# y00njaekim/CMU-11785-IDL-1.58bit-ASR

Hardware: AMD Instinct MI355X
Metric: mel-frames/sec (Conformer-S 1.58-bit train step) (higher is better)
Workload: dtype fp32; 1 GPU; conformer-s-1.58bit-train-step; global_batch=32, execution=hip-graph, per_gpu_batch=32, frames=1000, d_model=144, blocks=16, d_ff=576, heads=4, vocab=5004, parallelism=dp1, passes=teacher 2-bit + student 1-bit + SP, conv_pointwise=fp32 (reference)

## Files before the change

cmu-11785-idl-1.58bit-asr_amd/csrc/capi.hip:

```cpp
#include <algorithm>
#include <vector>

#include "../../include/onebit_hip.h"
#include "ob_launch.h"
#include <stdint.h>

using namespace ob;

namespace {

constexpr int kAbiVersion = 4;

inline hipStream_t as_stream(void* s) { return reinterpret_cast<hipStream_t>(s); }

inline bool aligned4(const void* p) { return (reinterpret_cast<uintptr_t>(p) & 3) == 0; }
inline bool misaligned8(const void* p) { return (reinterpret_cast<uintptr_t>(p) & 7) != 0; }

inline int check_bits(int bits) { return (bits == 1 || bits == 2) ? OB_OK : OB_ERR_BITWIDTH; }

inline int launched() {
  const hipError_t e = hipGetLastError();
  return e == hipSuccess ? OB_OK : OB_ERR_HIP;
}

// ... 970 lines not shown
}

size_t ob_dw_finish_entry_bytes(void) { return sizeof(DwFinishEntry); }

int ob_dw_finish_table(const void* table, int64_t n, int64_t total_blocks, void* stream) {
  if (n < 0 || total_blocks < 0 || total_blocks > 0x7fffffff) return OB_ERR_SHAPE;
  if (n > 0 && !table) return OB_ERR_NULL;
  launch_dw_finish_table(static_cast<const DwFinishEntry*>(table), (int)n, total_blocks,
                         as_stream(stream));
  return launched();
}

int ob_dw_grouped_supported(int64_t N, int64_t K) {
  return N > 0 && K > 0 && N % kDwgTile == 0 && K % kDwgTile == 0 && N <= (1 << 20) &&
         K <= (1 << 20);
}

namespace {
struct DwgPlan {
  std::vector<DwgDesc> d;
  int64_t steps = 0;
  int tiles = 0, blocks = 0;
  size_t table = 0, slots = 0, talpha = 0, total = 0;
};

int dwg_plan(const ob_dwg_gemm* g, int64_t G, DwgPlan& pl) {
  if (G < 1 || G > (1 << 16)) return OB_ERR_SHAPE;
  if (!g) return OB_ERR_NULL;
  pl.d.resize((size_t)G);
  int64_t tiles = 0;
  for (int64_t i = 0; i < G; ++i) {
    const ob_dwg_gemm& e = g[i];
    if (!ob_dw_grouped_supported(e.N, e.K) || e.M < 1 || e.P < 1 || e.P > kMaxPasses ||
        e.M * e.P >= ((int64_t)1 << 30) || e.M * std::max(e.N, e.K) * 4 >= ((int64_t)1 << 31) ||
        e.N * e.K * 4 >= ((int64_t)1 << 31))
      return OB_ERR_SHAPE;
    if (!e.dY || !e.X || !e.dW) return OB_ERR_NULL;
    if (e.W && (!e.alpha || !e.dalpha)) return OB_ERR_NULL;
    if (e.W && !e.pass_bits && check_bits(e.bits) != OB_OK) return OB_ERR_BITWIDTH;
    if (!aligned4(e.dY) || !aligned4(e.X) || ((reinterpret_cast<uintptr_t>(e.dY) |
                                               reinterpret_cast<uintptr_t>(e.X)) & 15))
      return OB_ERR_ALIGN;
    DwgDesc& d = pl.d[(size_t)i];
    d.dY = e.dY;
    d.X = e.X;
    d.W = e.W;
    d.alpha = e.alpha;
    d.pass_bits = e.pass_bits;
    d.dW = e.dW;
    d.db = e.db;
    d.dalpha = e.dalpha;
    d.N = (int)e.N;
    d.K = (int)e.K;
    d.Mp = (int)e.M;
    d.P = (int)e.P;
    d.alpha_raw = e.alpha_raw;
    d.bits = e.bits;
    d.spp = (int)ceil_div(e.M, 32);
    d.tiles_k = (int)(e.K / kDwgTile);
    d.tiles = (int)((e.N / kDwgTile) * d.tiles_k);
    d.tile0 = (int)tiles;
    d.work0 = pl.steps;
    tiles += d.tiles;
    pl.steps += (int64_t)d.tiles * d.P * d.spp;
  }
  if (tiles > (1 << 24) || pl.steps >= ((int64_t)1 << 31)) return OB_ERR_SHAPE;
  pl.tiles = (int)tiles;
  pl.blocks = dwg_blocks(pl.steps);
  pl.table = align_up(sizeof(DwgDesc) * (size_t)G);
  pl.slots = align_up(dwg_slot_bytes() * 2 * (size_t)pl.blocks);
  pl.talpha = align_up(sizeof(float) * (size_t)tiles);
  pl.total = pl.table + pl.slots + pl.talpha;
  return OB_OK;
}
}

size_t ob_dw_grouped_workspace(const ob_dwg_gemm* gemms, int64_t G) {
  DwgPlan pl;
  return dwg_plan(gemms, G, pl) == OB_OK ? pl.total : 0;
}

size_t ob_dw_grouped_tickets(const ob_dwg_gemm* gemms, int64_t G) {
  DwgPlan pl;
  return dwg_plan(gemms, G, pl) == OB_OK ? (size_t)pl.tiles + (size_t)G : 0;
}

int ob_dw_grouped(const ob_dwg_gemm* gemms, int64_t G, void* ws, size_t ws_bytes, void* tickets,
                  size_t ticket_words, void* stream) {
  DwgPlan pl;
  const int st = dwg_plan(gemms, G, pl);
  if (st != OB_OK) return st;
  if (!ws || !tickets) return OB_ERR_NULL;
  if (ws_bytes < pl.total || ticket_words < (size_t)pl.tiles + (size_t)G) return OB_ERR_WORKSPACE;
  unsigned char* base = static_cast<unsigned char*>(ws);
  launch_dw_grouped(pl.d.data(), (int)G, pl.steps, pl.blocks, reinterpret_cast<DwgDesc*>(base),
                    reinterpret_cast<float*>(base + pl.table),
                    reinterpret_cast<float*>(base + pl.table + pl.slots),
                    static_cast<uint32_t*>(tickets), pl.tiles, as_stream(stream));
  return launched();
}

int ob_dwconv1d_fwd(const float* x, const float* w, const float* bias, int64_t B, int64_t C,
                    int64_t T, int64_t KT, float* y, void* stream) {
  if (B < 0 || C < 0 || T < 0 || KT < 1 || KT % 2 == 0 || !dwconv_supported((int)KT))
    return OB_ERR_SHAPE;
  if (B * C * T > 0 && (!x || !y || !w)) return OB_ERR_NULL;
  if (!aligned4(x) || !aligned4(y) || !aligned4(w) || !aligned4(bias)) return OB_ERR_ALIGN;
// ... 1087 lines not shown
```

cmu-11785-idl-1.58bit-asr_amd/csrc/dw.hip:

```cpp
#include <cstdlib>
#include <type_traits>

#include "ob_launch.h"
#include "ob_mma.h"
#include "ob_quant.h"

namespace ob {

namespace {

constexpr int kThreads = 256;

constexpr int kDwTile = 64;

template <bool VEC, int S>
__global__ __launch_bounds__(kThreads) void dw_partial_kernel(
    const float* __restrict__ dY, const float* __restrict__ X, int64_t M, int64_t N, int64_t K,
    int64_t tiles_k, int64_t rows_per_chunk, int64_t cpp, float* __restrict__ part,
    float* __restrict__ part_db, uint32_t* __restrict__ ticket) {
  __shared__ float red[2][kDwTile * kDwTile];
  __shared__ float dbred[4][kDwTile];

  const int lane = threadIdx.x & 63;
  const int wave = threadIdx.x >> 6;
// ... 654 lines not shown
constexpr int kDwgAl = kDwgDb + kDwgTile;
constexpr unsigned kSc1 = 16;

__device__ __forceinline__ int dwg_start(int b, int nb, int W) {
  return (int)((long long)b * W / nb);
}
__device__ __forceinline__ int dwg_owner(int x, int nb, int W) {
  return (int)(((long long)(x + 1) * nb - 1) / W);
}

__device__ __forceinline__ float ld_f32(__amdgpu_buffer_rsrc_t r, int voff) {
  return __builtin_bit_cast(float, __builtin_amdgcn_raw_buffer_load_b32(r, voff, 0, 0));
}
__device__ __forceinline__ void st_f32(float v, __amdgpu_buffer_rsrc_t r, int voff) {
  __builtin_amdgcn_raw_buffer_store_b32(__builtin_bit_cast(uint32_t, v), r, voff, 0, 0);
}

__device__ __forceinline__ int opaque(int x) {
  asm volatile("" : "+v"(x));
  return x;
}

constexpr int kDwgWaves = 8, kDwgThreads = 64 * kDwgWaves;
constexpr int kDwgBuf = 2 * kDwgTile * kLdsPitch;
constexpr int kDwgLds = 2 * kDwgBuf + 16 * kDwgTile * 4 + 16;

__global__ __launch_bounds__(kDwgThreads) void dw_grouped_kernel(
    const DwgDesc* __restrict__ descs, int G, int Wtot, float* __restrict__ slots,
    float* __restrict__ talpha, uint32_t* __restrict__ tickets, int total_tiles) {
  constexpr int BN = kDwgTile;
  extern __shared__ __attribute__((aligned(16))) unsigned char lds[];
  const int lane = threadIdx.x & 63;
  const int wave = __builtin_amdgcn_readfirstlane(threadIdx.x >> 6);
  const int bn = wave / 3, bk = wave - 3 * bn;
  const int tie = 6 + bn, tue = 6 + bk;
  const bool two = wave == 7;
  const int r = lane & 15, g = lane >> 4;
  const int nb = gridDim.x, blk = blockIdx.x;
  const int beg = dwg_start(blk, nb, Wtot), end = dwg_start(blk + 1, nb, Wtot);
  float* const s_db = reinterpret_cast<float*>(lds + 2 * kDwgBuf);
  int* const s_flag = reinterpret_cast<int*>(lds + 2 * kDwgBuf + 16 * kDwgTile * 4);
  float* const fl = reinterpret_cast<float*>(lds);
  const bool u2 = wave == 0;
  const int rp0 = threadIdx.x & 15, cq0 = 4 * (threadIdx.x >> 4);
  const int cq1 = 128 + cq0;

  int gi = 0;
  {
    int lo = 0, hi = G - 1;
    while (lo < hi) {
      const int mid = (lo + hi + 1) >> 1;
      if (descs[mid].work0 <= beg) lo = mid;
      else hi = mid - 1;
    }
    gi = lo;
  }

  auto put = [&](unsigned char* base, int col, const f32x4& r0, const f32x4& r1) {
#pragma unroll
    for (int e = 0; e < 4; ++e) {
      uint32_t ph, pm, pl;
      split2(r0[e], r1[e], ph, pm, pl);
      unsigned char* cb = base + (col + e) * kLdsPitch + rp0 * 4;
      *reinterpret_cast<uint32_t*>(cb) = ph;
      *reinterpret_cast<uint32_t*>(cb + 64) = pm;
      *reinterpret_cast<uint32_t*>(cb + 128) = pl;
    }
  };
  auto frag = [&](const unsigned char* base, int col, int plane) {
    return *reinterpret_cast<const bf16x8*>(base + col * kLdsPitch + 64 * plane + 16 * g);
  };

  int pos = beg;
  while (pos < end) {
    const DwgDesc& d = descs[gi];
    const int tsteps = d.P * d.spp;
    if (pos >= (int)d.work0 + tsteps * d.tiles) {
      ++gi;
      continue;
    }
    const int t = (pos - (int)d.work0) / tsteps;
    const int T0 = (int)d.work0 + t * tsteps, T1 = T0 + tsteps;
    const int send = end < T1 ? end : T1;
    const int N = d.N, K = d.K, Mp = d.Mp, spp = d.spp;
    const int tn = t / d.tiles_k, tk = t - tn * d.tiles_k;
    const int n0 = tn * kDwgTile, k0 = tk * kDwgTile;
    const bool has_al = d.W != nullptr;
    const bool do_db = d.db != nullptr && tk == 0;
    const float a = has_al ? effective_alpha(d.alpha, d.alpha_raw) : 1.0f;
    const __amdgpu_buffer_rsrc_t rw = make_rsrc(d.W, has_al ? (int64_t)N * K * 4 : 0);
    auto pass_bits = [&](int p) {
      const int b = d.pass_bits ? d.pass_bits[p] : d.bits;
      return b == 1 ? 1 : 2;
    };

    f32x4 acc[3][3], acce[2];
#pragma unroll
    for (int i = 0; i < 3; ++i)
#pragma unroll
      for (int u = 0; u < 3; ++u) acc[i][u] = f32x4{0.f, 0.f, 0.f, 0.f};
    acce[0] = acce[1] = f32x4{0.f, 0.f, 0.f, 0.f};
    auto for_tiles = [&](auto&& fn) {
#pragma unroll
      for (int i = 0; i < 3; ++i)
#pragma unroll
        for (int u = 0; u < 3; ++u) fn(acc[i][u], 3 * bn + i, 3 * bk + u);
      fn(acce[0], tie, tue);
      if (two) fn(acce[1], 8, 8);
    };
    auto elem_base = [&]() {
      const int ln = opaque(lane);
      return ((n0 + 4 * (ln >> 4)) * K + k0 + (ln & 15)) * 4;
    };
    float aprod = 0.0f;
    auto alpha_dot = [&](int b1, int b2) {
      const int eb = elem_base();
      for_tiles([&](f32x4& ac, int ti, int tu) {
        float w[4];
#pragma unroll
        for (int reg = 0; reg < 4; ++reg)
          w[reg] = ld_f32(rw, eb + ((16 * ti + reg) * K + 16 * tu) * 4);
#pragma unroll
        for (int reg = 0; reg < 4; ++reg) {
          const float wa = w[reg] / a;
          aprod += ac[reg] * (alpha_term(wa, b1) - (b2 ? alpha_term(wa, b2) : 0.0f));
        }
      });
    };
    f32x4* const db0 = reinterpret_cast<f32x4*>(s_db + rp0 * kDwgTile + cq0);
    f32x4* const db1 = reinterpret_cast<f32x4*>(s_db + rp0 * kDwgTile + cq1);

    __syncthreads();
    if (do_db) {
      *db0 = f32x4{0.f, 0.f, 0.f, 0.f};
      if (u2) *db1 = f32x4{0.f, 0.f, 0.f, 0.f};
    }
    int j = pos - T0;
    const int j1 = send - T0;
    while (j < j1) {
      const int p = j / spp;
      const int je = j1 < (p + 1) * spp ? j1 : (p + 1) * spp;
      const int r0 = p * Mp + (j - p * spp) * kStepRows;
      const int rl = p * Mp + (je - p * spp) * kStepRows;
      const int r1 = rl < (p + 1) * Mp ? rl : (p + 1) * Mp;
      const int steps = je - j;
      const __amdgpu_buffer_rsrc_t ry =
          make_rsrc(d.dY + (int64_t)r0 * N, (int64_t)(r1 - r0) * N * 4);
      const __amdgpu_buffer_rsrc_t rx =
          make_rsrc(d.X + (int64_t)r0 * K, (int64_t)(r1 - r0) * K * 4);
      const __amdgpu_buffer_rsrc_t ry2 = u2 ? ry : make_rsrc(d.dY, 0);
      const __amdgpu_buffer_rsrc_t rx2 = u2 ? rx : make_rsrc(d.X, 0);
      const int yv0 = (2 * rp0 * N + n0 + cq0) * 4, xv0 = (2 * rp0 * K + k0 + cq0) * 4;
      struct Raw {
        f32x4 y[2][2];
        f32x4 x[2][2];
      };
      auto load = [&](Raw& raw, int step) {
        const int soy = step * kStepRows * N * 4, sox = step * kStepRows * K * 4;
#pragma unroll
        for (int i = 0; i < 2; ++i) {
          raw.y[0][i] = __builtin_amdgcn_raw_buffer_load_b128(ry, yv0, soy + i * N * 4, 0);
          raw.x[0][i] = __builtin_amdgcn_raw_buffer_load_b128(rx, xv0, sox + i * K * 4, 0);
        }
#pragma unroll
        for (int i = 0; i < 2; ++i) {
          raw.y[1][i] = __builtin_amdgcn_raw_buffer_load_b128(ry2, yv0 + 512, soy + i * N * 4, 0);
          raw.x[1][i] = __builtin_amdgcn_raw_buffer_load_b128(rx2, xv0 + 512, sox + i * K * 4, 0);
        }
      };
      auto store = [&](const Raw& raw, int buf) {
        unsigned char* base = lds + buf * kDwgBuf;
        if (do_db) *db0 = *db0 + (raw.y[0][0] + raw.y[0][1]);
        put(base, cq0, raw.y[0][0], raw.y[0][1]);
        put(base, BN + cq0, raw.x[0][0], raw.x[0][1]);
        if (u2) {
          if (do_db) *db1 = *db1 + (raw.y[1][0] + raw.y[1][1]);
          put(base, cq1, raw.y[1][0], raw.y[1][1]);
          put(base, BN + cq1, raw.x[1][0], raw.x[1][1]);
        }
      };
      auto compute = [&](int buf) {
        const unsigned char* base = lds + buf * kDwgBuf;
        bf16x8 bq[3][3];
#pragma unroll
        for (int u = 0; u < 3; ++u)
#pragma unroll
          for (int q = 0; q < 3; ++q) bq[u][q] = frag(base, BN + 48 * bk + 16 * u + r, q);
#pragma unroll
        for (int i = 0; i < 3; ++i) {
          bf16x8 aq[3];
#pragma unroll
          for (int q = 0; q < 3; ++q) aq[q] = frag(base, 48 * bn + 16 * i + r, q);
#pragma unroll
          for (int pr = 0; pr < 6; ++pr)
#pragma unroll
            for (int u = 0; u < 3; ++u)
              acc[i][u] = mfma_bf16(aq[kProdA[pr]], bq[u][kProdB[pr]], acc[i][u]);
        }
        bf16x8 ae[3], be[3];
#pragma unroll
        for (int q = 0; q < 3; ++q) ae[q] = frag(base, 16 * tie + r, q);
#pragma unroll
        for (int q = 0; q < 3; ++q) be[q] = frag(base, BN + 16 * tue + r, q);
#pragma unroll
        for (int pr = 0; pr < 6; ++pr) acce[0] = mfma_bf16(ae[kProdA[pr]], be[kProdB[pr]], acce[0]);
        if (two) {
#pragma unroll
          for (int q = 0; q < 3; ++q) be[q] = frag(base, BN + 16 * 8 + r, q);
#pragma unroll
          for (int pr = 0; pr < 6; ++pr)
            acce[1] = mfma_bf16(ae[kProdA[pr]], be[kProdB[pr]], acce[1]);
        }
      };
      auto phase = [&](int cb, Raw& nxt, int sb, bool do_store, int ld_step) {
        (void)do_store;
        store(nxt, sb);
        compute(cb);
        load(nxt, ld_step);
      };
      Raw ra, rb;
      load(ra, 0);
      load(rb, 1);
      store(ra, 0);
      load(ra, 2);
      __syncthreads();
      for (int s = 0; s < steps; s += 2) {
        phase(0, rb, 1, true, s + 3);
        __syncthreads();
        phase(1, ra, 0, true, s + 4);
        __syncthreads();
      }
      if (has_al) {
        const int bp = pass_bits(p);
        if (je == j1) {
          alpha_dot(bp, 0);
        } else {
          const int bq = pass_bits(p + 1);
          if (bq != bp) alpha_dot(bp, bq);
        }
      }
      j = je;
    }

    const int tid = opaque((int)threadIdx.x);
    const int ln = tid & 63;
    if (has_al) {
#pragma unroll
      for (int off = 32; off >= 1; off >>= 1) aprod += __shfl_xor(aprod, off, 64);
      if (ln == 0) fl[wave] = aprod;
    }
    __syncthreads();
    float dbv = 0.0f, ap = 0.0f;
    if (do_db && tid < kDwgTile) {
#pragma unroll
      for (int q = 0; q < 16; ++q) dbv += s_db[q * kDwgTile + tid];
    }
    if (has_al && tid == 0) {
      for (int w = 0; w < kDwgWaves; ++w) ap += fl[w];
    }
    auto slab_off = [&](int ti, int tu) { return ((ti * 9 + tu) * 64) * 16; };

    bool finish = pos == T0 && send == T1;
    if (!finish) {
      const int nsl = dwg_owner(T1 - 1, nb, Wtot) - dwg_owner(T0, nb, Wtot) + 1;
      float* slab = slots + (int64_t)(2 * blk + (beg >= T0 ? 0 : 1)) * kDwgSlotF;
      const __amdgpu_buffer_rsrc_t rs = make_rsrc(slab, (int64_t)kDwgSlotF * 4);
      for_tiles([&](f32x4& ac, int ti, int tu) {
        __builtin_amdgcn_raw_buffer_store_b128(ac, rs, ln * 16, slab_off(ti, tu), kSc1);
      });
      if (do_db && tid < kDwgTile)
        __hip_atomic_store(slab + kDwgDb + tid, dbv, __ATOMIC_RELAXED, __HIP_MEMORY_SCOPE_AGENT);
      if (has_al && tid == 0)
        __hip_atomic_store(slab + kDwgAl, ap, __ATOMIC_RELAXED, __HIP_MEMORY_SCOPE_AGENT);
      asm volatile("s_waitcnt vmcnt(0)" ::: "memory");
      __syncthreads();
      if (tid == 0) {
        const uint32_t old = __hip_atomic_fetch_add(tickets + d.tile0 + t, 1u, __ATOMIC_RELAXED,
                                                    __HIP_MEMORY_SCOPE_AGENT);
        *s_flag = old == (uint32_t)(nsl - 1);
      }
      __syncthreads();
      finish = *s_flag != 0;
      if (finish) {
        __builtin_amdgcn_fence(__ATOMIC_ACQUIRE, "wavefront");
        const int bf = dwg_owner(T0, nb, Wtot);
        dbv = 0.0f;
        ap = 0.0f;
        for (int q = 0; q < nsl; ++q) {
          const int bb = bf + q;
          const float* sl =
              slots + (int64_t)(2 * bb + (dwg_start(bb, nb, Wtot) >= T0 ? 0 : 1)) * kDwgSlotF;
          const __amdgpu_buffer_rsrc_t rl = make_rsrc(sl, (int64_t)kDwgSlotF * 4);
          for_tiles([&](f32x4& ac, int ti, int tu) {
            const f32x4 v = __builtin_amdgcn_raw_buffer_load_b128(rl, ln * 16, slab_off(ti, tu), kSc1);
            ac = q == 0 ? v : ac + v;
          });
          if (do_db && tid < kDwgTile) {
            const float v =
                __hip_atomic_load(sl + kDwgDb + tid, __ATOMIC_RELAXED, __HIP_MEMORY_SCOPE_AGENT);
            dbv = q == 0 ? v : dbv + v;
          }
          if (has_al && tid == 0) {
            const float v =
                __hip_atomic_load(sl + kDwgAl, __ATOMIC_RELAXED, __HIP_MEMORY_SCOPE_AGENT);
            ap = q == 0 ? v : ap + v;
          }
        }
        if (tid == 0)
          __hip_atomic_store(tickets + d.tile0 + t, 0u, __ATOMIC_RELAXED, __HIP_MEMORY_SCOPE_AGENT);
      }
    }
    if (finish) {
      const __amdgpu_buffer_rsrc_t rd = make_rsrc(d.dW, (int64_t)N * K * 4);
      const int eb = elem_base();
      for_tiles([&](f32x4& ac, int ti, int tu) {
        float w[4];
        if (has_al) {
#pragma unroll
          for (int reg = 0; reg < 4; ++reg)
            w[reg] = ld_f32(rw, eb + ((16 * ti + reg) * K + 16 * tu) * 4);
        }
#pragma unroll
        for (int reg = 0; reg < 4; ++reg) {
          float v = ac[reg];
          if (has_al) v *= ste_indicator(w[reg] / a);
          st_f32(v, rd, eb + ((16 * ti + reg) * K + 16 * tu) * 4);
        }
      });
      if (do_db && tid < kDwgTile) d.db[n0 + tid] = dbv;
      if (has_al && tid == 0) {
        const float chain = alpha_chain(d.alpha, d.alpha_raw);
        if (d.tiles == 1) {
          *d.dalpha = ap * chain;
        } else {
          __hip_atomic_store(talpha + d.tile0 + t, ap, __ATOMIC_RELAXED, __HIP_MEMORY_SCOPE_AGENT);
          asm volatile("s_waitcnt vmcnt(0)" ::: "memory");
          uint32_t* gt = tickets + total_tiles + gi;
          const uint32_t old =
              __hip_atomic_fetch_add(gt, 1u, __ATOMIC_RELAXED, __HIP_MEMORY_SCOPE_AGENT);
          if (old == (uint32_t)(d.tiles - 1)) {
            __builtin_amdgcn_fence(__ATOMIC_ACQUIRE, "wavefront");
            float s2 = 0.0f;
            for (int q = 0; q < d.tiles; ++q)
              s2 += __hip_atomic_load(talpha + d.tile0 + q, __ATOMIC_RELAXED,
                                      __HIP_MEMORY_SCOPE_AGENT);
            *d.dalpha = s2 * chain;
            __hip_atomic_store(gt, 0u, __ATOMIC_RELAXED, __HIP_MEMORY_SCOPE_AGENT);
          }
        }
      }
    }
    pos = send;
  }
}

constexpr int kDwgChunk = 32;
static_assert(sizeof(DwgDesc) * kDwgChunk + 64 <= 4096, "dwg_table_kernel arguments exceed 4 KiB");
struct DwgChunk {
  DwgDesc d[kDwgChunk];
};
__global__ void dwg_table_kernel(DwgDesc* table, int off, int n, DwgChunk c) {
  if ((int)threadIdx.x < n) table[off + threadIdx.x] = c.d[threadIdx.x];
}


}

DwPlan plan_dw(int64_t M, int64_t N, int64_t K) { return plan_dw_passes(1, M, N, K); }

DwPlan plan_dw_passes(int64_t P, int64_t Mp, int64_t N, int64_t K) {
  DwPlan p;
  const int64_t M = P * Mp;
  if (N % 4 != 0 || K % 4 != 0 || N < 4 || K < 4) {
    p.variant = 0;
    p.tiles_n = N > 0 ? ceil_div(N, kDwTile) : 1;
// ... 116 lines not shown
                   dW, db, dalpha};
  const int64_t nb = finish_blocks(a);
  hipLaunchKernelGGL(dw_finish_kernel, dim3((unsigned)nb), dim3(kThreads), 0, s, a);
}

int64_t dw_finish_blocks(const DwFinish& a) { return finish_blocks(a); }

__global__ void dw_table_entry_kernel(DwFinishEntry* table, int slot, DwFinishEntry ent) {
  table[slot] = ent;
}

void launch_dw_table_entry(DwFinishEntry* table, int slot, const DwFinishEntry& ent,
                           hipStream_t s) {
  hipLaunchKernelGGL(dw_table_entry_kernel, dim3(1), dim3(1), 0, s, table, slot, ent);
}

void launch_dw_finish_table(const DwFinishEntry* table, int n, int64_t total_blocks,
                            hipStream_t s) {
  if (n <= 0 || total_blocks <= 0) return;
  hipLaunchKernelGGL(dw_finish_table_kernel, dim3((unsigned)total_blocks), dim3(kThreads), 0, s,
                     table, n, total_blocks);
}

int dwg_blocks(int64_t total_steps) {
  int dev = 0, cus = 0;
  if (hipGetDevice(&dev) != hipSuccess ||
      hipDeviceGetAttribute(&cus, hipDeviceAttributeMultiprocessorCount, dev) != hipSuccess ||
      cus <= 0)
    cus = 256;
  return (int)(total_steps < cus ? total_steps : cus);
}

size_t dwg_slot_bytes() { return sizeof(float) * (size_t)kDwgSlotF; }

void launch_dw_grouped(const DwgDesc* host_descs, int G, int64_t total_steps, int blocks,
                       DwgDesc* table, float* slots, float* talpha, uint32_t* tickets,
                       int total_tiles, hipStream_t s) {
  for (int off = 0; off < G; off += kDwgChunk) {
    DwgChunk c{};
    const int n = G - off < kDwgChunk ? G - off : kDwgChunk;
    for (int i = 0; i < n; ++i) c.d[i] = host_descs[off + i];
    hipLaunchKernelGGL(dwg_table_kernel, dim3(1), dim3(kDwgChunk), 0, s, table, off, n, c);
  }
  hipLaunchKernelGGL(dw_grouped_kernel, dim3((unsigned)blocks), dim3(kDwgThreads),
                     (size_t)kDwgLds, s, table, G, (int)total_steps, slots,
                     talpha, tickets, total_tiles);
}

void launch_dw_finish_group(const DwFinish* a, int n, hipStream_t s) {
  DwFinishGroup G{};
  G.n = n;
  int64_t total = 0;
  for (int i = 0; i < n; ++i) {
    G.g[i] = a[i];
    G.start[i] = (int)total;
    total += finish_blocks(a[i]);
// ... 14 lines not shown
```

cmu-11785-idl-1.58bit-asr_amd/csrc/ob_launch.h:

```cpp
#pragma once

#include <hip/hip_runtime.h>
#include <stddef.h>
#include <stdint.h>

#include "../../include/onebit_hip.h"

namespace ob {

inline int64_t ceil_div(int64_t a, int64_t b) { return (a + b - 1) / b; }

void launch_quant_pack(const float* W, const float* alpha, int alpha_raw, int bits,
                       const int* bits_dev, int64_t N, int64_t K, uint32_t* codes,
                       uint32_t* codes_t, hipStream_t s);
int64_t quant_pack_item_blocks(int64_t N, int64_t K);
int64_t quant_pack_item_blocks16(int64_t N, int64_t K);
void launch_quant_pack_group(const ob_pack_item* items_dev, int n_items, int64_t total_blocks,
                             hipStream_t s);
void launch_quant_dequant(const float* W, const float* alpha, int alpha_raw, int bits, int64_t n,
                          float* W_hat, hipStream_t s);

int64_t ste_reduce_blocks(int64_t total);
void launch_ste_reduce(const float* part, int chunks, int64_t nk, const float* part_db,
                       int64_t n_db, const float* W, const float* alpha, int alpha_raw, int bits,
// ... 157 lines not shown
};
int64_t dw_finish_blocks(const DwFinish& a);
void launch_dw_table_entry(DwFinishEntry* table, int slot, const DwFinishEntry& ent, hipStream_t s);
void launch_dw_finish_table(const DwFinishEntry* table, int n, int64_t total_blocks, hipStream_t s);
void launch_dw_partial_group_defer(const float* const* dY, int G, const float* X, int64_t M,
                                   int64_t N, int64_t K, const DwPlan& p, float* const* part,
                                   float* const* part_db, const DwAlpha* al,
                                   DwFinishEntry* table, int slot, const DwFinishEntry* ent,
                                   hipStream_t s);

struct DwgDesc {
  const float* dY;
  const float* X;
  const float* W;
  const float* alpha;
  const int* pass_bits;
  float* dW;
  float* db;
  float* dalpha;
  int64_t work0;
  int N, K, Mp, P, alpha_raw, bits;
  int spp;
  int tiles_k;
  int tiles;
  int tile0;
};
constexpr int kDwgTile = 144;
int dwg_blocks(int64_t total_steps);
size_t dwg_slot_bytes();
void launch_dw_grouped(const DwgDesc* host_descs, int G, int64_t total_steps, int blocks,
                       DwgDesc* table, float* slots, float* talpha, uint32_t* tickets,
                       int total_tiles, hipStream_t s);

bool dense_gemm_supported(int64_t K, int64_t N);
struct DenseEpi {
  const float* R;
  float p_drop;
  const uint64_t* rng;
  uint64_t rng_off;
};
bool launch_dense_gemm(const float* A, int64_t M, int64_t K, const float* W, int trans,
                       const float* bias, int64_t N, float* C, hipStream_t s,
                       const DenseEpi* epi = nullptr);

bool ternary_gemm_i8_supported(int64_t K, int64_t N);
void launch_silu_monotone_check(uint32_t lo, uint32_t hi, uint32_t* bad, hipStream_t s);
size_t act_absmax_workspace(int P);
void launch_act_absmax(const float* X, int P, int64_t n_per_pass, float* amax, void* ws,
                       hipStream_t s);
void launch_act_dequant(const float* X, int P, int64_t n_per_pass, const float* amax, float* Xd,
                        hipStream_t s);
// ... 261 lines not shown
```

cmu-11785-idl-1.58bit-asr_amd/onebit_asr/_lib.py:

```python
from __future__ import annotations

import ctypes
import os
from pathlib import Path

import torch

LIB_NAME = "libonebit_hip.so"
LIB_PATH = Path(os.environ.get("ONEBIT_HIP_LIB") or Path(__file__).with_name(LIB_NAME))

OB_OK = 0
OB_ERR_SHAPE = -2
OB_ERR_BITWIDTH = -3

_c_f = ctypes.c_void_p
_i64 = ctypes.c_int64
_int = ctypes.c_int
_sz = ctypes.c_size_t
_f32 = ctypes.c_float
_f64 = ctypes.c_double

SIGNATURES = {
    "ob_abi_version": (_int, []),
    "ob_source_digest": (ctypes.c_char_p, []),
# ... 177 lines not shown
    "ob_layernorm_fwd_i8": (_int, [_c_f, _c_f, _c_f, _i64, _i64, _f32, _i64, _c_f, _c_f, _c_f,
                                   _sz, _c_f]),
    "ob_layernorm_bwd_defer": (
        _int, [_c_f, _c_f, _c_f, _c_f, _c_f, _i64, _i64, _c_f, _c_f, _c_f, _c_f, _c_f, _sz, _c_f,
               _f32, _f32, _c_f, _i64, _c_f, _i64, _c_f, _i64, _c_f]),
    "ob_layernorm_bwd_pair_workspace": (_sz, [_i64, _i64]),
    "ob_layernorm_bwd_pair": (
        _int, [_c_f, _c_f, _c_f, _c_f, _c_f, _c_f, _c_f, _c_f, _c_f, _c_f, _i64, _i64, _c_f, _c_f,
               _c_f, _c_f, _c_f, _c_f, _sz, _c_f, _f32, _f32, _c_f, _i64, _c_f, _i64, _c_f, _i64,
               _i64, _c_f]),
    "ob_ln_param_entry_bytes": (_sz, []),
    "ob_ln_param_table": (_int, [_c_f, _i64, _i64, _c_f]),
    "ob_dw_finish_entry_bytes": (_sz, []),
    "ob_bitlinear_bwd_dw_passes_defer": (
        _int, [_c_f, _c_f, _i64, _i64, _i64, _i64, _c_f, _c_f, _int, _c_f, _c_f, _c_f, _c_f, _c_f,
               _sz, _c_f, _i64, _i64, _c_f, _c_f]),
    "ob_bitlinear_bwd_dw_passes_group_defer": (
        _int, [_i64, _c_f, _c_f, _i64, _i64, _i64, _i64, _c_f, _c_f, _int, _c_f, _c_f, _c_f, _c_f,
               _c_f, _sz, _c_f, _i64, _i64, _c_f, _c_f]),
    "ob_dw_finish_table": (_int, [_c_f, _i64, _i64, _c_f]),
    "ob_dw_grouped_supported": (_int, [_i64, _i64]),
    "ob_dw_grouped_workspace": (_sz, [_c_f, _i64]),
    "ob_dw_grouped_tickets": (_sz, [_c_f, _i64]),
    "ob_dw_grouped": (_int, [_c_f, _i64, _c_f, _sz, _c_f, _sz, _c_f]),
    "ob_dense_dw_defer": (_int, [_c_f, _c_f, _i64, _i64, _i64, _c_f, _c_f, _c_f, _sz, _c_f, _i64,
                                 _i64, _c_f, _c_f]),
    "ob_layernorm_bwd_workspace": (_sz, [_i64, _i64]),
    "ob_layernorm_bwd": (
        _int, [_c_f, _c_f, _c_f, _c_f, _c_f, _i64, _i64, _c_f, _c_f, _c_f, _c_f, _sz, _c_f]),
    "ob_layernorm_bwd_res": (
        _int, [_c_f, _c_f, _c_f, _c_f, _c_f, _i64, _i64, _c_f, _c_f, _c_f, _c_f, _c_f, _sz, _c_f]),
    "ob_layernorm_bwd_ex": (
        _int, [_c_f, _c_f, _c_f, _c_f, _c_f, _i64, _i64, _c_f, _c_f, _c_f, _c_f, _c_f, _sz, _c_f,
               _f32, _f32, _c_f, _i64, _c_f, _i64, _c_f]),
    "ob_act_absmax_workspace": (_sz, [_i64]),
    "ob_act_absmax": (_int, [_c_f, _i64, _i64, _c_f, _c_f, _sz, _c_f]),
    "ob_act_dequant_i8": (_int, [_c_f, _i64, _i64, _c_f, _c_f, _c_f]),
    "ob_bitlinear_fwd_i8": (
        _int, [_c_f, _i64, _i64, _i64, _c_f, _c_f, _c_f, _c_f, _int, _c_f, _c_f, _i64, _c_f, _c_f]),
    "ob_bitlinear_fwd_i8_epi": (
        _int, [_c_f, _i64, _i64, _i64, _c_f, _c_f, _c_f, _c_f, _int, _c_f, _c_f, _i64, _int, _c_f,
               _f32, _c_f, _i64, _c_f, _c_f, _c_f]),
    "ob_bitlinear_fwd_passes_group": (
        _int, [_i64, _c_f, _i64, _i64, _i64, _c_f, _c_f, _c_f, _c_f, _int, _c_f, _i64, _c_f, _c_f]),
    "ob_bitlinear_fwd_i8q": (
        _int, [_c_f, _i64, _i64, _i64, _c_f, _c_f, _c_f, _c_f, _int, _c_f, _c_f, _i64, _int, _c_f,
# ... 108 lines not shown
```

include/onebit_hip.h:

```cpp
#ifndef ONEBIT_HIP_H_
#define ONEBIT_HIP_H_

#include <stddef.h>
#include <stdint.h>

#ifdef __cplusplus
extern "C" {
#endif

#define OB_API __attribute__((visibility("default")))

enum {
  OB_OK = 0,
  OB_ERR_NULL = -1,
  OB_ERR_SHAPE = -2,
  OB_ERR_BITWIDTH = -3,
  OB_ERR_WORKSPACE = -4,
  OB_ERR_ALIGN = -5,
  OB_ERR_HIP = -6
};

OB_API int ob_abi_version(void);
OB_API const char* ob_source_digest(void);
OB_API const char* ob_status_string(int status);
// ... 177 lines not shown
OB_API int ob_bitlinear_bwd_dw_passes_group_defer(
    int64_t G, const float* const* dY, const float* X, int64_t P, int64_t M, int64_t N,
    int64_t K, const float* const* W, const float* const* alpha, int alpha_raw,
    const int32_t* pass_bits, float* const* dW, float* const* dalpha, float* const* db,
    void* ws, size_t ws_bytes, void* table, int64_t slot, int64_t start, int64_t* n_blocks,
    void* stream);
OB_API int ob_dw_finish_table(const void* table, int64_t n, int64_t total_blocks, void* stream);

typedef struct ob_dwg_gemm {
  const float* dY;
  const float* X;
  const float* W;
  const float* alpha;
  const int32_t* pass_bits;
  float* dW;
  float* db;
  float* dalpha;
  int64_t N, K, M, P;
  int32_t alpha_raw, bits;
} ob_dwg_gemm;
OB_API int ob_dw_grouped_supported(int64_t N, int64_t K);
OB_API size_t ob_dw_grouped_workspace(const ob_dwg_gemm* gemms, int64_t G);
OB_API size_t ob_dw_grouped_tickets(const ob_dwg_gemm* gemms, int64_t G);
OB_API int ob_dw_grouped(const ob_dwg_gemm* gemms, int64_t G, void* ws, size_t ws_bytes,
                         void* tickets, size_t ticket_words, void* stream);

OB_API int ob_decattn_supported(int64_t Lq, int64_t Lk, int64_t dh);
OB_API int ob_decattn_fwd(const float* q, int64_t sq, const float* k, int64_t sk, const float* v,
                          int64_t sv, const uint8_t* kmask, int64_t causal, int64_t B, int64_t H,
                          int64_t Lq, int64_t Lk, int64_t dh, float p_drop, const int64_t* rng,
                          int64_t rng_offset, float* probs, float* ctx, void* stream);
OB_API int ob_decattn_bwd(const float* dctx, const float* ctx, const float* q, int64_t sq,
                          const float* k, int64_t sk, const float* v, int64_t sv, int64_t B, int64_t H, int64_t Lq,
                          int64_t Lk, int64_t dh, float p_drop, float* probs, float* dq,
                          int64_t gq, float* dk, int64_t gk, float* dv, int64_t gv, void* stream);
OB_API int ob_decattn_fwd_grouped(const float* q, int64_t sq, const float* k, int64_t sk,
                                  const float* v, int64_t sv, const uint8_t* kmask,
                                  int64_t causal, int64_t B, int64_t kv_group, int64_t H,
                                  int64_t Lq, int64_t Lk, int64_t dh, float* ctx, void* stream);

OB_API int ob_relattn_fwd(const float* q, const float* k, const float* v, const float* pos,
                          const float* u, const float* vb, const int32_t* lens, int64_t Bt,
                          int64_t P, int64_t T, int64_t H, int64_t d, float p_drop,
                          const int64_t* rng, int64_t rng_offset, float* saved, float* probs,
                          float* ctx, void* stream);
OB_API int64_t ob_relattn_saved_elems(int64_t Bt, int64_t T, int64_t H, int64_t d);
// ... 322 lines not shown
```

Baseline: 1.408 million mel-frames/s.

## Pair adjacent dW output tiles in grouped kernel to share one operand load

The grouped weight-gradient kernel now processes pairs of adjacent 144x144 output tiles, along N or along K, as one work unit. The shared operand (X or dY) is loaded into LDS once and reused for both tiles, so each pair streams three operand panels instead of four. This costs a second set of accumulators, double-size split-K slots and bias reduction buffers, more syncs per step, and coarser work units for load balancing. A helper reports the operand bytes read.

```diff
diff --git a/cmu-11785-idl-1.58bit-asr_amd/csrc/capi.hip b/cmu-11785-idl-1.58bit-asr_amd/csrc/capi.hip
--- a/cmu-11785-idl-1.58bit-asr_amd/csrc/capi.hip
+++ b/cmu-11785-idl-1.58bit-asr_amd/csrc/capi.hip
@@ -1016,6 +1016,7 @@
   int64_t steps = 0;
   int tiles = 0, blocks = 0;
   size_t table = 0, slots = 0, talpha = 0, total = 0;
+  size_t operand_bytes = 0;
 };
 
 int dwg_plan(const ob_dwg_gemm* g, int64_t G, DwgPlan& pl) {
@@ -1052,15 +1053,22 @@
     d.bits = e.bits;
     d.spp = (int)ceil_div(e.M, 32);
     d.tiles_k = (int)(e.K / kDwgTile);
-    d.tiles = (int)((e.N / kDwgTile) * d.tiles_k);
+    const DwgPairing pr = dwg_pairing(e.N, e.K);
+    d.pairs = pr.pairs;
+    d.singles = pr.singles;
+    d.kdir = pr.kdir;
     d.tile0 = (int)tiles;
     d.work0 = pl.steps;
-    tiles += d.tiles;
-    pl.steps += (int64_t)d.tiles * d.P * d.spp;
+    const int64_t gt = 2 * (int64_t)pr.pairs + pr.singles;
+    tiles += gt;
+    pl.steps += gt * d.P * d.spp;
+    pl.steps += pl.steps & 1;
+    pl.operand_bytes += (size_t)e.M * e.P * 4 *
+                        ((size_t)pr.pairs * 3 * kDwgTile + (size_t)pr.singles * 2 * kDwgTile);
   }
   if (tiles > (1 << 24) || pl.steps >= ((int64_t)1 << 31)) return OB_ERR_SHAPE;
   pl.tiles = (int)tiles;
-  pl.blocks = dwg_blocks(pl.steps);
+  pl.blocks = dwg_blocks(pl.steps / 2);
   pl.table = align_up(sizeof(DwgDesc) * (size_t)G);
   pl.slots = align_up(dwg_slot_bytes() * 2 * (size_t)pl.blocks);
   pl.talpha = align_up(sizeof(float) * (size_t)tiles);
@@ -1077,6 +1085,11 @@
 size_t ob_dw_grouped_tickets(const ob_dwg_gemm* gemms, int64_t G) {
   DwgPlan pl;
   return dwg_plan(gemms, G, pl) == OB_OK ? (size_t)pl.tiles + (size_t)G : 0;
+}
+
+size_t ob_dw_grouped_operand_bytes(const ob_dwg_gemm* gemms, int64_t G) {
+  DwgPlan pl;
+  return dwg_plan(gemms, G, pl) == OB_OK ? pl.operand_bytes : 0;
 }
 
 int ob_dw_grouped(const ob_dwg_gemm* gemms, int64_t G, void* ws, size_t ws_bytes, void* tickets,
diff --git a/cmu-11785-idl-1.58bit-asr_amd/csrc/dw.hip b/cmu-11785-idl-1.58bit-asr_amd/csrc/dw.hip
--- a/cmu-11785-idl-1.58bit-asr_amd/csrc/dw.hip
+++ b/cmu-11785-idl-1.58bit-asr_amd/csrc/dw.hip
@@ -700,13 +700,17 @@
 }
 
 constexpr int kDwgWaves = 8, kDwgThreads = 64 * kDwgWaves;
-constexpr int kDwgBuf = 2 * kDwgTile * kLdsPitch;
-constexpr int kDwgLds = 2 * kDwgBuf + 16 * kDwgTile * 4 + 16;
+constexpr int kDwgReg = kDwgTile * kLdsPitch;
+constexpr int kDwgBuf = 2 * kDwgReg;
+constexpr int kDwgDbF = 16 * kDwgTile;
+constexpr int kDwgLds = 2 * kDwgBuf + 2 * kDwgDbF * 4 + 16;
 
 __global__ __launch_bounds__(kDwgThreads) void dw_grouped_kernel(
     const DwgDesc* __restrict__ descs, int G, int Wtot, float* __restrict__ slots,
     float* __restrict__ talpha, uint32_t* __restrict__ tickets, int total_tiles) {
   constexpr int BN = kDwgTile;
+  using C0 = std::integral_constant<int, 0>;
+  using C1 = std::integral_constant<int, 1>;
   extern __shared__ __attribute__((aligned(16))) unsigned char lds[];
   const int lane = threadIdx.x & 63;
   const int wave = __builtin_amdgcn_readfirstlane(threadIdx.x >> 6);
@@ -715,9 +719,10 @@
   const bool two = wave == 7;
   const int r = lane & 15, g = lane >> 4;
   const int nb = gridDim.x, blk = blockIdx.x;
-  const int beg = dwg_start(blk, nb, Wtot), end = dwg_start(blk + 1, nb, Wtot);
+  const int H = Wtot >> 1;
+  const int beg = 2 * dwg_start(blk, nb, H), end = 2 * dwg_start(blk + 1, nb, H);
   float* const s_db = reinterpret_cast<float*>(lds + 2 * kDwgBuf);
-  int* const s_flag = reinterpret_cast<int*>(lds + 2 * kDwgBuf + 16 * kDwgTile * 4);
+  int* const s_flag = reinterpret_cast<int*>(lds + 2 * kDwgBuf + 2 * kDwgDbF * 4);
   float* const fl = reinterpret_cast<float*>(lds);
   const bool u2 = wave == 0;
   const int rp0 = threadIdx.x & 15, cq0 = 4 * (threadIdx.x >> 4);
@@ -753,18 +758,42 @@
   while (pos < end) {
     const DwgDesc& d = descs[gi];
     const int tsteps = d.P * d.spp;
-    if (pos >= (int)d.work0 + tsteps * d.tiles) {
+    const int work0 = (int)d.work0;
+    const int pw = 2 * d.pairs * tsteps;
+    if (pos >= work0 + pw + d.singles * tsteps) {
+      if (gi + 1 >= G) break;
       ++gi;
       continue;
     }
-    const int t = (pos - (int)d.work0) / tsteps;
-    const int T0 = (int)d.work0 + t * tsteps, T1 = T0 + tsteps;
+    if (pos < work0) {
+      pos = work0;
+      continue;
+    }
+    auto run_unit = [&](auto pair_c) -> int {
+    constexpr bool pair = decltype(pair_c)::value;
+    const int cost = pair ? 2 : 1;
+    const int t = pair ? (pos - work0) / (2 * tsteps) : d.pairs + (pos - work0 - pw) / tsteps;
+    const int T0 = pair ? work0 + t * 2 * tsteps : work0 + pw + (t - d.pairs) * tsteps;
+    const int T1 = T0 + cost * tsteps;
     const int send = end < T1 ? end : T1;
     const int N = d.N, K = d.K, Mp = d.Mp, spp = d.spp;
-    const int tn = t / d.tiles_k, tk = t - tn * d.tiles_k;
+    const bool kdir = d.kdir != 0;
+    const int tiles_n = N / kDwgTile;
+    int tn, tk;
+    if (pair) {
+      const int pn = kdir ? 1 : tiles_n / 2;
+      tk = kdir ? 2 * t : t / pn;
+      tn = kdir ? 0 : 2 * (t - tk * pn);
+    } else {
+      tn = kdir ? 0 : tiles_n - 1;
+      tk = kdir ? d.tiles_k - 1 : t - d.pairs;
+    }
+    const int units = d.pairs + d.singles;
     const int n0 = tn * kDwgTile, k0 = tk * kDwgTile;
+    const int n0b = n0 + (kdir ? 0 : kDwgTile), k0b = k0 + (kdir ? kDwgTile : 0);
     const bool has_al = d.W != nullptr;
     const bool do_db = d.db != nullptr && tk == 0;
+    const bool do_dbb = do_db && pair && !kdir;
     const float a = has_al ? effective_alpha(d.alpha, d.alpha_raw) : 1.0f;
     const __amdgpu_buffer_rsrc_t rw = make_rsrc(d.W, has_al ? (int64_t)N * K * 4 : 0);
     auto pass_bits = [&](int p) {
@@ -772,38 +801,45 @@
       return b == 1 ? 1 : 2;
     };
 
-    f32x4 acc[3][3], acce[2];
-#pragma unroll
-    for (int i = 0; i < 3; ++i)
-#pragma unroll
-      for (int u = 0; u < 3; ++u) acc[i][u] = f32x4{0.f, 0.f, 0.f, 0.f};
-    acce[0] = acce[1] = f32x4{0.f, 0.f, 0.f, 0.f};
-    auto for_tiles = [&](auto&& fn) {
+    f32x4 acc[2][3][3], acce[2][2];
+#pragma unroll
+    for (int w = 0; w < 2; ++w) {
 #pragma unroll
       for (int i = 0; i < 3; ++i)
 #pragma unroll
-        for (int u = 0; u < 3; ++u) fn(acc[i][u], 3 * bn + i, 3 * bk + u);
-      fn(acce[0], tie, tue);
-      if (two) fn(acce[1], 8, 8);
+        for (int u = 0; u < 3; ++u) acc[w][i][u] = f32x4{0.f, 0.f, 0.f, 0.f};
+      acce[w][0] = acce[w][1] = f32x4{0.f, 0.f, 0.f, 0.f};
+    }
+    auto for_tiles = [&](auto wc, auto&& fn) {
+      constexpr int w = decltype(wc)::value;
+#pragma unroll
+      for (int i = 0; i < 3; ++i)
+#pragma unroll
+        for (int u = 0; u < 3; ++u) fn(acc[w][i][u], 3 * bn + i, 3 * bk + u);
+      fn(acce[w][0], tie, tue);
+      if (two) fn(acce[w][1], 8, 8);
     };
-    auto elem_base = [&]() {
+    auto elem_base = [&](int tn0, int tk0) {
       const int ln = opaque(lane);
-      return ((n0 + 4 * (ln >> 4)) * K + k0 + (ln & 15)) * 4;
+      return ((tn0 + 4 * (ln >> 4)) * K + tk0 + (ln & 15)) * 4;
     };
     float aprod = 0.0f;
     auto alpha_dot = [&](int b1, int b2) {
-      const int eb = elem_base();
-      for_tiles([&](f32x4& ac, int ti, int tu) {
-        float w[4];
-#pragma unroll
-        for (int reg = 0; reg < 4; ++reg)
-          w[reg] = ld_f32(rw, eb + ((16 * ti + reg) * K + 16 * tu) * 4);
-#pragma unroll
-        for (int reg = 0; reg < 4; ++reg) {
-          const float wa = w[reg] / a;
-          aprod += ac[reg] * (alpha_term(wa, b1) - (b2 ? alpha_term(wa, b2) : 0.0f));
-        }
-      });
+      auto one = [&](auto wc, int eb) {
+        for_tiles(wc, [&](f32x4& ac, int ti, int tu) {
+          float w[4];
+#pragma unroll
+          for (int reg = 0; reg < 4; ++reg)
+            w[reg] = ld_f32(rw, eb + ((16 * ti + reg) * K + 16 * tu) * 4);
+#pragma unroll
+          for (int reg = 0; reg < 4; ++reg) {
+            const float wa = w[reg] / a;
+            aprod += ac[reg] * (alpha_term(wa, b1) - (b2 ? alpha_term(wa, b2) : 0.0f));
+          }
+        });
+      };
+      one(C0{}, elem_base(n0, k0));
+      if (pair) one(C1{}, elem_base(n0b, k0b));
     };
     f32x4* const db0 = reinterpret_cast<f32x4*>(s_db + rp0 * kDwgTile + cq0);
     f32x4* const db1 = reinterpret_cast<f32x4*>(s_db + rp0 * kDwgTile + cq1);
@@ -813,8 +849,12 @@
       *db0 = f32x4{0.f, 0.f, 0.f, 0.f};
       if (u2) *db1 = f32x4{0.f, 0.f, 0.f, 0.f};
     }
-    int j = pos - T0;
-    const int j1 = send - T0;
+    if (do_dbb) {
+      db0[kDwgDbF / 4] = f32x4{0.f, 0.f, 0.f, 0.f};
+      if (u2) db1[kDwgDbF / 4] = f32x4{0.f, 0.f, 0.f, 0.f};
+    }
+    int j = (pos - T0) / cost;
+    const int j1 = (send - T0) / cost;
     while (j < j1) {
       const int p = j / spp;
       const int je = j1 < (p + 1) * spp ? j1 : (p + 1) * spp;
@@ -857,56 +897,131 @@
           put(base, BN + cq1, raw.x[1][0], raw.x[1][1]);
         }
       };
-      auto compute = [&](int buf) {
-        const unsigned char* base = lds + buf * kDwgBuf;
+      auto compute = [&](auto wc, const unsigned char* ya, const unsigned char* xa) {
+        constexpr int w = decltype(wc)::value;
         bf16x8 bq[3][3];
 #pragma unroll
         for (int u = 0; u < 3; ++u)
 #pragma unroll
-          for (int q = 0; q < 3; ++q) bq[u][q] = frag(base, BN + 48 * bk + 16 * u + r, q);
+          for (int q = 0; q < 3; ++q) bq[u][q] = frag(xa, 48 * bk + 16 * u + r, q);
 #pragma unroll
         for (int i = 0; i < 3; ++i) {
           bf16x8 aq[3];
 #pragma unroll
-          for (int q = 0; q < 3; ++q) aq[q] = frag(base, 48 * bn + 16 * i + r, q);
+          for (int q = 0; q < 3; ++q) aq[q] = frag(ya, 48 * bn + 16 * i + r, q);
 #pragma unroll
           for (int pr = 0; pr < 6; ++pr)
 #pragma unroll
             for (int u = 0; u < 3; ++u)
-              acc[i][u] = mfma_bf16(aq[kProdA[pr]], bq[u][kProdB[pr]], acc[i][u]);
+              acc[w][i][u] = mfma_bf16(aq[kProdA[pr]], bq[u][kProdB[pr]], acc[w][i][u]);
         }
         bf16x8 ae[3], be[3];
 #pragma unroll
-        for (int q = 0; q < 3; ++q) ae[q] = frag(base, 16 * tie + r, q);
-#pragma unroll
-        for (int q = 0; q < 3; ++q) be[q] = frag(base, BN + 16 * tue + r, q);
-#pragma unroll
-        for (int pr = 0; pr < 6; ++pr) acce[0] = mfma_bf16(ae[kProdA[pr]], be[kProdB[pr]], acce[0]);
+        for (int q = 0; q < 3; ++q) ae[q] = frag(ya, 16 * tie + r, q);
+#pragma unroll
+        for (int q = 0; q < 3; ++q) be[q] = frag(xa, 16 * tue + r, q);
+#pragma unroll
+        for (int pr = 0; pr < 6; ++pr)
+          acce[w][0] = mfma_bf16(ae[kProdA[pr]], be[kProdB[pr]], acce[w][0]);
         if (two) {
 #pragma unroll
-          for (int q = 0; q < 3; ++q) be[q] = frag(base, BN + 16 * 8 + r, q);
+          for (int q = 0; q < 3; ++q) be[q] = frag(xa, 16 * 8 + r, q);
 #pragma unroll
           for (int pr = 0; pr < 6; ++pr)
-            acce[1] = mfma_bf16(ae[kProdA[pr]], be[kProdB[pr]], acce[1]);
+            acce[w][1] = mfma_bf16(ae[kProdA[pr]], be[kProdB[pr]], acce[w][1]);
         }
       };
       auto phase = [&](int cb, Raw& nxt, int sb, bool do_store, int ld_step) {
         (void)do_store;
         store(nxt, sb);
-        compute(cb);
+        compute(C0{}, lds + cb * kDwgBuf, lds + cb * kDwgBuf + kDwgReg);
         load(nxt, ld_step);
       };
-      Raw ra, rb;
-      load(ra, 0);
-      load(rb, 1);
-      store(ra, 0);
-      load(ra, 2);
-      __syncthreads();
-      for (int s = 0; s < steps; s += 2) {
-        phase(0, rb, 1, true, s + 3);
+      if (!pair) {
+        Raw ra, rb;
+        load(ra, 0);
+        load(rb, 1);
+        store(ra, 0);
+        load(ra, 2);
         __syncthreads();
-        phase(1, ra, 0, true, s + 4);
+        for (int s = 0; s < steps; s += 2) {
+          phase(0, rb, 1, true, s + 3);
+          __syncthreads();
+          phase(1, ra, 0, true, s + 4);
+          __syncthreads();
+        }
+      } else {
+        const int lds_s = kdir ? N : K, ldt = kdir ? K : N;
+        const float* const sp = kdir ? d.dY : d.X;
+        const float* const tp = kdir ? d.X : d.dY;
+        const __amdgpu_buffer_rsrc_t rs =
+            make_rsrc(sp + (int64_t)r0 * lds_s, (int64_t)(r1 - r0) * lds_s * 4);
+        const __amdgpu_buffer_rsrc_t rt =
+            make_rsrc(tp + (int64_t)r0 * ldt, (int64_t)(r1 - r0) * ldt * 4);
+        const __amdgpu_buffer_rsrc_t rs2 = u2 ? rs : make_rsrc(sp, 0);
+        const __amdgpu_buffer_rsrc_t rt2 = u2 ? rt : make_rsrc(tp, 0);
+        const int sv0 = kdir ? yv0 : xv0, tv0 = kdir ? xv0 : yv0;
+        struct R4 {
+          f32x4 v[2][2];
+        };
+        auto load4 = [&](R4& q, __amdgpu_buffer_rsrc_t d1, __amdgpu_buffer_rsrc_t d2, int voff,
+                         int ld, int step) {
+          const int so = step * kStepRows * ld * 4;
+#pragma unroll
+          for (int i = 0; i < 2; ++i)
+            q.v[0][i] = __builtin_amdgcn_raw_buffer_load_b128(d1, voff, so + i * ld * 4, 0);
+#pragma unroll
+          for (int i = 0; i < 2; ++i)
+            q.v[1][i] = __builtin_amdgcn_raw_buffer_load_b128(d2, voff + 512, so + i * ld * 4, 0);
+        };
+        auto store4 = [&](const R4& q, unsigned char* base, int dbo) {
+          if (dbo >= 0) db0[dbo / 4] = db0[dbo / 4] + (q.v[0][0] + q.v[0][1]);
+          put(base, cq0, q.v[0][0], q.v[0][1]);
+          if (u2) {
+            if (dbo >= 0) db1[dbo / 4] = db1[dbo / 4] + (q.v[1][0] + q.v[1][1]);
+            put(base, cq1, q.v[1][0], q.v[1][1]);
+          }
+        };
+        const int db_s = kdir && do_db ? 0 : -1;
+        const int db_ta = !kdir && do_db ? 0 : -1;
+        const int db_tb = !kdir && do_db ? kDwgDbF : -1;
+        unsigned char* const reg_ta = lds + 2 * kDwgReg;
+        unsigned char* const reg_tb = lds + 3 * kDwgReg;
+        constexpr int kTb = kDwgTile * 4;
+        R4 qa, qb0, qb1, qs;
+        auto half_a = [&](int sb, R4& qb, int ld_step) {
+          unsigned char* const sh = lds + sb * kDwgReg;
+          store4(qb, reg_tb, db_tb);
+          compute(C0{}, kdir ? sh : reg_ta, kdir ? reg_ta : sh);
+          load4(qb, rt, rt2, tv0 + kTb, ldt, ld_step);
+        };
+        auto half_b = [&](int sb, int ld_step) {
+          unsigned char* const sh = lds + sb * kDwgReg;
+          store4(qa, reg_ta, db_ta);
+          store4(qs, lds + (sb ^ 1) * kDwgReg, db_s);
+          compute(C1{}, kdir ? sh : reg_tb, kdir ? reg_tb : sh);
+          load4(qa, rt, rt2, tv0, ldt, ld_step);
+          load4(qs, rs, rs2, sv0, lds_s, ld_step);
+        };
+        load4(qa, rt, rt2, tv0, ldt, 0);
+        load4(qs, rs, rs2, sv0, lds_s, 0);
+        load4(qb0, rt, rt2, tv0 + kTb, ldt, 0);
+        store4(qa, reg_ta, db_ta);
+        store4(qs, lds, db_s);
+        load4(qa, rt, rt2, tv0, ldt, 1);
+        load4(qs, rs, rs2, sv0, lds_s, 1);
+        load4(qb1, rt, rt2, tv0 + kTb, ldt, 1);
         __syncthreads();
+        for (int s = 0; s < steps; s += 2) {
+          half_a(0, qb0, s + 2);
+          __syncthreads();
+          half_b(0, s + 2);
+          __syncthreads();
+          half_a(1, qb1, s + 3);
+          __syncthreads();
+          half_b(1, s + 3);
+          __syncthreads();
+        }
       }
       if (has_al) {
         const int bp = pass_bits(p);
@@ -928,26 +1043,42 @@
       if (ln == 0) fl[wave] = aprod;
     }
     __syncthreads();
-    float dbv = 0.0f, ap = 0.0f;
+    float dbv = 0.0f, dbvb = 0.0f, ap = 0.0f;
     if (do_db && tid < kDwgTile) {
 #pragma unroll
       for (int q = 0; q < 16; ++q) dbv += s_db[q * kDwgTile + tid];
+    }
+    if (do_dbb && tid < kDwgTile) {
+#pragma unroll
+      for (int q = 0; q < 16; ++q) dbvb += s_db[kDwgDbF + q * kDwgTile + tid];
     }
     if (has_al && tid == 0) {
       for (int w = 0; w < kDwgWaves; ++w) ap += fl[w];
     }
     auto slab_off = [&](int ti, int tu) { return ((ti * 9 + tu) * 64) * 16; };
+    auto unit_slot = [&](int b, int which) {
+      return slots + (int64_t)(2 * b + which) * (2 * kDwgSlotF);
+    };
 
     bool finish = pos == T0 && send == T1;
     if (!finish) {
-      const int nsl = dwg_owner(T1 - 1, nb, Wtot) - dwg_owner(T0, nb, Wtot) + 1;
-      float* slab = slots + (int64_t)(2 * blk + (beg >= T0 ? 0 : 1)) * kDwgSlotF;
+      const int nsl = dwg_owner((T1 - 1) >> 1, nb, H) - dwg_owner(T0 >> 1, nb, H) + 1;
+      float* slab = unit_slot(blk, beg >= T0 ? 0 : 1);
       const __amdgpu_buffer_rsrc_t rs = make_rsrc(slab, (int64_t)kDwgSlotF * 4);
-      for_tiles([&](f32x4& ac, int ti, int tu) {
+      for_tiles(C0{}, [&](f32x4& ac, int ti, int tu) {
         __builtin_amdgcn_raw_buffer_store_b128(ac, rs, ln * 16, slab_off(ti, tu), kSc1);
       });
+      if (pair) {
+        const __amdgpu_buffer_rsrc_t rsb = make_rsrc(slab + kDwgSlotF, (int64_t)kDwgSlotF * 4);
+        for_tiles(C1{}, [&](f32x4& ac, int ti, int tu) {
+          __builtin_amdgcn_raw_buffer_store_b128(ac, rsb, ln * 16, slab_off(ti, tu), kSc1);
+        });
+      }
       if (do_db && tid < kDwgTile)
         __hip_atomic_store(slab + kDwgDb + tid, dbv, __ATOMIC_RELAXED, __HIP_MEMORY_SCOPE_AGENT);
+      if (do_dbb && tid < kDwgTile)
+        __hip_atomic_store(slab + kDwgSlotF + kDwgDb + tid, dbvb, __ATOMIC_RELAXED,
+                           __HIP_MEMORY_SCOPE_AGENT);
       if (has_al && tid == 0)
         __hip_atomic_store(slab + kDwgAl, ap, __ATOMIC_RELAXED, __HIP_MEMORY_SCOPE_AGENT);
       asm volatile("s_waitcnt vmcnt(0)" ::: "memory");
@@ -961,22 +1092,35 @@
       finish = *s_flag != 0;
       if (finish) {
         __builtin_amdgcn_fence(__ATOMIC_ACQUIRE, "wavefront");
-        const int bf = dwg_owner(T0, nb, Wtot);
+        const int bf = dwg_owner(T0 >> 1, nb, H);
         dbv = 0.0f;
+        dbvb = 0.0f;
         ap = 0.0f;
         for (int q = 0; q < nsl; ++q) {
           const int bb = bf + q;
-          const float* sl =
-              slots + (int64_t)(2 * bb + (dwg_start(bb, nb, Wtot) >= T0 ? 0 : 1)) * kDwgSlotF;
+          const float* sl = unit_slot(bb, 2 * dwg_start(bb, nb, H) >= T0 ? 0 : 1);
           const __amdgpu_buffer_rsrc_t rl = make_rsrc(sl, (int64_t)kDwgSlotF * 4);
-          for_tiles([&](f32x4& ac, int ti, int tu) {
+          for_tiles(C0{}, [&](f32x4& ac, int ti, int tu) {
             const f32x4 v = __builtin_amdgcn_raw_buffer_load_b128(rl, ln * 16, slab_off(ti, tu), kSc1);
             ac = q == 0 ? v : ac + v;
           });
+          if (pair) {
+            const __amdgpu_buffer_rsrc_t rlb = make_rsrc(sl + kDwgSlotF, (int64_t)kDwgSlotF * 4);
+            for_tiles(C1{}, [&](f32x4& ac, int ti, int tu) {
+              const f32x4 v =
+                  __builtin_amdgcn_raw_buffer_load_b128(rlb, ln * 16, slab_off(ti, tu), kSc1);
+              ac = q == 0 ? v : ac + v;
+            });
+          }
           if (do_db && tid < kDwgTile) {
             const float v =
                 __hip_atomic_load(sl + kDwgDb + tid, __ATOMIC_RELAXED, __HIP_MEMORY_SCOPE_AGENT);
             dbv = q == 0 ? v : dbv + v;
+          }
+          if (do_dbb && tid < kDwgTile) {
+            const float v = __hip_atomic_load(sl + kDwgSlotF + kDwgDb + tid, __ATOMIC_RELAXED,
+                                              __HIP_MEMORY_SCOPE_AGENT);
+            dbvb = q == 0 ? v : dbvb + v;
           }
           if (has_al && tid == 0) {
             const float v =
@@ -990,25 +1134,29 @@
     }
     if (finish) {
       const __amdgpu_buffer_rsrc_t rd = make_rsrc(d.dW, (int64_t)N * K * 4);
-      const int eb = elem_base();
-      for_tiles([&](f32x4& ac, int ti, int tu) {
-        float w[4];
-        if (has_al) {
-#pragma unroll
-          for (int reg = 0; reg < 4; ++reg)
-            w[reg] = ld_f32(rw, eb + ((16 * ti + reg) * K + 16 * tu) * 4);
-        }
-#pragma unroll
-        for (int reg = 0; reg < 4; ++reg) {
-          float v = ac[reg];
-          if (has_al) v *= ste_indicator(w[reg] / a);
-          st_f32(v, rd, eb + ((16 * ti + reg) * K + 16 * tu) * 4);
-        }
-      });
+      auto write_tile = [&](auto wc, int eb) {
+        for_tiles(wc, [&](f32x4& ac, int ti, int tu) {
+          float w[4];
+          if (has_al) {
+#pragma unroll
+            for (int reg = 0; reg < 4; ++reg)
+              w[reg] = ld_f32(rw, eb + ((16 * ti + reg) * K + 16 * tu) * 4);
+          }
+#pragma unroll
+          for (int reg = 0; reg < 4; ++reg) {
+            float v = ac[reg];
+            if (has_al) v *= ste_indicator(w[reg] / a);
+            st_f32(v, rd, eb + ((16 * ti + reg) * K + 16 * tu) * 4);
+          }
+        });
+      };
+      write_tile(C0{}, elem_base(n0, k0));
+      if (pair) write_tile(C1{}, elem_base(n0b, k0b));
       if (do_db && tid < kDwgTile) d.db[n0 + tid] = dbv;
+      if (do_dbb && tid < kDwgTile) d.db[n0b + tid] = dbvb;
       if (has_al && tid == 0) {
         const float chain = alpha_chain(d.alpha, d.alpha_raw);
-        if (d.tiles == 1) {
+        if (units == 1) {
           *d.dalpha = ap * chain;
         } else {
           __hip_atomic_store(talpha + d.tile0 + t, ap, __ATOMIC_RELAXED, __HIP_MEMORY_SCOPE_AGENT);
@@ -1016,10 +1164,10 @@
           uint32_t* gt = tickets + total_tiles + gi;
           const uint32_t old =
               __hip_atomic_fetch_add(gt, 1u, __ATOMIC_RELAXED, __HIP_MEMORY_SCOPE_AGENT);
-          if (old == (uint32_t)(d.tiles - 1)) {
+          if (old == (uint32_t)(units - 1)) {
             __builtin_amdgcn_fence(__ATOMIC_ACQUIRE, "wavefront");
             float s2 = 0.0f;
-            for (int q = 0; q < d.tiles; ++q)
+            for (int q = 0; q < units; ++q)
               s2 += __hip_atomic_load(talpha + d.tile0 + q, __ATOMIC_RELAXED,
                                       __HIP_MEMORY_SCOPE_AGENT);
             *d.dalpha = s2 * chain;
@@ -1028,7 +1176,9 @@
         }
       }
     }
-    pos = send;
+    return send;
+    };
+    pos = pos - work0 < pw ? run_unit(std::true_type{}) : run_unit(std::false_type{});
   }
 }
 
@@ -1191,16 +1341,16 @@
                      table, n, total_blocks);
 }
 
-int dwg_blocks(int64_t total_steps) {
+int dwg_blocks(int64_t pair_steps) {
   int dev = 0, cus = 0;
   if (hipGetDevice(&dev) != hipSuccess ||
       hipDeviceGetAttribute(&cus, hipDeviceAttributeMultiprocessorCount, dev) != hipSuccess ||
       cus <= 0)
     cus = 256;
-  return (int)(total_steps < cus ? total_steps : cus);
-}
-
-size_t dwg_slot_bytes() { return sizeof(float) * (size_t)kDwgSlotF; }
+  return (int)(pair_steps < cus ? pair_steps : cus);
+}
+
+size_t dwg_slot_bytes() { return sizeof(float) * 2 * (size_t)kDwgSlotF; }
 
 void launch_dw_grouped(const DwgDesc* host_descs, int G, int64_t total_steps, int blocks,
                        DwgDesc* table, float* slots, float* talpha, uint32_t* tickets,
diff --git a/cmu-11785-idl-1.58bit-asr_amd/csrc/ob_launch.h b/cmu-11785-idl-1.58bit-asr_amd/csrc/ob_launch.h
--- a/cmu-11785-idl-1.58bit-asr_amd/csrc/ob_launch.h
+++ b/cmu-11785-idl-1.58bit-asr_amd/csrc/ob_launch.h
@@ -203,11 +203,20 @@
   int N, K, Mp, P, alpha_raw, bits;
   int spp;
   int tiles_k;
-  int tiles;
   int tile0;
+  int pairs, singles, kdir;
 };
 constexpr int kDwgTile = 144;
-int dwg_blocks(int64_t total_steps);
+struct DwgPairing {
+  int pairs, singles, kdir;
+};
+inline DwgPairing dwg_pairing(int64_t N, int64_t K) {
+  const int tn = (int)(N / kDwgTile), tk = (int)(K / kDwgTile);
+  if (tn >= 2) return {(tn / 2) * tk, (tn % 2) * tk, 0};
+  if (tk >= 2) return {tk / 2, tk % 2, 1};
+  return {0, 1, 0};
+}
+int dwg_blocks(int64_t pair_steps);
 size_t dwg_slot_bytes();
 void launch_dw_grouped(const DwgDesc* host_descs, int G, int64_t total_steps, int blocks,
                        DwgDesc* table, float* slots, float* talpha, uint32_t* tickets,
diff --git a/cmu-11785-idl-1.58bit-asr_amd/onebit_asr/_lib.py b/cmu-11785-idl-1.58bit-asr_amd/onebit_asr/_lib.py
--- a/cmu-11785-idl-1.58bit-asr_amd/onebit_asr/_lib.py
+++ b/cmu-11785-idl-1.58bit-asr_amd/onebit_asr/_lib.py
@@ -223,6 +223,7 @@
     "ob_dw_grouped_supported": (_int, [_i64, _i64]),
     "ob_dw_grouped_workspace": (_sz, [_c_f, _i64]),
     "ob_dw_grouped_tickets": (_sz, [_c_f, _i64]),
+    "ob_dw_grouped_operand_bytes": (_sz, [_c_f, _i64]),
     "ob_dw_grouped": (_int, [_c_f, _i64, _c_f, _sz, _c_f, _sz, _c_f]),
     "ob_dense_dw_defer": (_int, [_c_f, _c_f, _i64, _i64, _i64, _c_f, _c_f, _c_f, _sz, _c_f, _i64,
                                  _i64, _c_f, _c_f]),
diff --git a/include/onebit_hip.h b/include/onebit_hip.h
--- a/include/onebit_hip.h
+++ b/include/onebit_hip.h
@@ -223,6 +223,7 @@
 OB_API int ob_dw_grouped_supported(int64_t N, int64_t K);
 OB_API size_t ob_dw_grouped_workspace(const ob_dwg_gemm* gemms, int64_t G);
 OB_API size_t ob_dw_grouped_tickets(const ob_dwg_gemm* gemms, int64_t G);
+OB_API size_t ob_dw_grouped_operand_bytes(const ob_dwg_gemm* gemms, int64_t G);
 OB_API int ob_dw_grouped(const ob_dwg_gemm* gemms, int64_t G, void* ws, size_t ws_bytes,
                          void* tickets, size_t ticket_words, void* stream);
 
```

After: 1.422 million mel-frames/s, median of 6. No clear change (+0.9%).
